# elenasolano/CS87Project-msolano2

Measured on AMD Instinct MI355X. Metric: GFLOP/s (5N·log2N/t) + % HBM roofline, fp64 complex N=2^28 @1/2/4/8 GPU, higher is better.
Workload: dtype f64; 1 GPU; config 4: one fp64 complex N=2^28 pi-FFT, P=1 workers, 1 per GPU (no data-path collective); n=268435456, workers=1, workers_per_gpu=1, batch=1, batch_per_gpu=1, local_n=268435456, passes=3, parallelism=pi-split p1 over 1 GPU(s), full=False, detail=not written: PermissionError(13, 'Permission denied')

## Files before the change

cs87project-msolano2_amd/csrc/pifft.hip:

```cpp
#ifndef _GNU_SOURCE
#define _GNU_SOURCE
#endif
#include "pifft_gather.h"
#include "pifft_kernels.h"
#include "pifft_planner.h"
#include "pifft_real.h"
#include "pifft_table.h"
#include "../../include/pifft.h"

#include <hip/hip_ext.h>
#include <hip/hip_runtime.h>

#include <math.h>
#include <stdio.h>
#include <stdlib.h>
#include <string.h>

#include <cxxabi.h>

#include <algorithm>
#include <atomic>
#include <mutex>
#include <string>
#include <vector>

using namespace pifft;

namespace {

#define HIPCHK(expr)                                                                       \
    do {                                                                                   \
        hipError_t e_ = (expr);                                                            \
        if (e_ != hipSuccess) return fail("%s failed: %s", #expr, hipGetErrorString(e_)); \
    } while (0)

bool fault_at(const char* site) {
    if (!tuning_on()) return false;
    const char* s = getenv("PIFFT_FAULT");
    const size_t n = strlen(site);
    if (!s || strncmp(s, site, n)) return false;
// ... 130 lines not shown
enum { BUF_IN = 0, BUF_OUT = 1, BUF_W = 2, BUF_TA = 3, BUF_Z = 4, NBUF = 5 };

constexpr size_t kNoTable = (size_t)-1;
struct StepTables {
    size_t r = kNoTable, lo = kNoTable, hi = kNoTable;
    size_t tree_direct = kNoTable, tree_lo = kNoTable, tree_hi = kNoTable;
};

struct Step {
    int kind = 0;
    const void* fn = nullptr;
    const PassKernel* pk = nullptr;
    dim3 grid, block;
    size_t lds = 0;
    int src = -1, dst = -2;
    uint64_t src_off = 0, dst_off = 0;
    PassArgs pa{};
    int nts = 0;
    TreeArgs ta{};
    uint64_t il_total = 0;
    uint32_t il_log_n = 0, il_log_p = 0;
    RealArgs ra{};
    StepTables tab;
    uint64_t bytes = 0;
};

}

struct pifft_plan : pifft::PlanShape {
    int device = 0, flags = 0;
    bool ilv = false;
    bool wil = false;
    bool inverse = false;
    int real = 0;
    uint64_t real_n = 0;
    size_t bytes_z = 0;
    size_t rtw_bytes = 0;
    std::vector<Step> steps;
    int tree_steps = 0, npasses = 0;
    bool fused_tree = false;
    std::vector<Step> tree_only;
    std::vector<hipEvent_t> prof_ev;
#ifdef PIFFT_WG_CLOCK
    unsigned long long* dbg_clk = nullptr;
#endif
    int prof_steps = 0, prof_used = 0, prof_mode = 0;
    int radix[8] = {0}, lines[8] = {0}, vpt[8] = {0};
    void* buf[NBUF] = {nullptr};
    size_t bytes_w = 0, bytes_ta = 0;
    void* d_tw = nullptr;
    size_t tw_bytes = 0;
    hipStream_t stream = nullptr;
    std::vector<hipEvent_t> ev;
    hipEvent_t sev[3] = {nullptr, nullptr, nullptr};
    void* d_hin = nullptr;
    void* d_hout = nullptr;
    void* d_gather = nullptr;
    std::vector<char> host_tmp;
    std::vector<int> peer_on;
    std::vector<hipStream_t> gst;
    std::vector<hipEvent_t> gdone;
    hipEvent_t gev[2] = {nullptr, nullptr};
};

namespace {

// ... 113 lines not shown
    for (auto e : p->gev)
        if (e) (void)hipEventDestroy(e);
    for (auto e : p->ev) (void)hipEventDestroy(e);
    for (auto e : p->sev)
        if (e) (void)hipEventDestroy(e);
    for (auto e : p->prof_ev) (void)hipEventDestroy(e);
    if (p->stream) (void)hipStreamDestroy(p->stream);
    delete p;
}


struct TableLayout {
    size_t tree_direct = kNoTable;
    TwoLevel tree2;
    std::vector<size_t> tw_r;
    TwoLevel pass2;
};

TableLayout layout_tables(const PlanShape& s, const PlanChoice& ch, TableBuilder& tb) {
    TableLayout tl;
    if (ch.tree_tw == TREE_TW_DIRECT || ch.tree_tw == TREE_TW_WIL_FACTORED)
        tl.tree_direct = tb.reference_omega_levels(s.n, s.lp);
    if (ch.tree_tw == TREE_TW_FACTORED || ch.tree_tw == TREE_TW_WIL_FACTORED) tl.tree2 = two_level(tb, s.n);
    tl.tw_r.resize(ch.passes.size());
    for (size_t i = 0; i < ch.passes.size(); i++) {
        size_t found = kNoTable;
        for (size_t j = 0; j < i; j++)
            if (ch.passes[j]->R == ch.passes[i]->R) found = tl.tw_r[j];
        tl.tw_r[i] = (found != kNoTable) ? found : tb.roots(ch.passes[i]->R, ch.passes[i]->R, 1);
    }
    if (ch.passes.size() > 1) tl.pass2 = two_level(tb, s.m);
    tb.align();
    return tl;
}

int assemble_steps(pifft_plan* p, const PlanChoice& ch, const TableLayout& tl) {
    const size_t esz = p->esz;
    const uint64_t ntrans = (uint64_t)p->batch * p->nq;
    const size_t npass = ch.passes.size();
    const bool need_tree = p->P > 1;
    const bool fused = ch.fused != FUSED_NONE;
    p->wil = ch.wil;
    p->ilv = ch.ilv;
    p->fused_tree = fused;
    TreeTw ttw{};
    if (need_tree) {
        ttw.h = tl.tree2.h;
        ttw.log_n = (uint32_t)p->log_n;
    }
    auto tree_tables = [&](Step& s, bool wil) {
        const bool direct = tl.tree_direct != kNoTable && !(wil && ch.tree_tw == TREE_TW_WIL_FACTORED);
        s.tab.tree_direct = direct ? tl.tree_direct : kNoTable;
        s.tab.tree_lo = direct ? kNoTable : tl.tree2.lo;
        s.tab.tree_hi = direct ? kNoTable : tl.tree2.hi;
    };

    std::vector<std::vector<Step>> chain;
    const uint64_t M = p->m;
    if (need_tree) {
        std::vector<Step> e;
        static const void* tk64[5] = {nullptr, (const void*)&k_tree<double, 1>, (const void*)&k_tree<double, 2>,
                                      (const void*)&k_tree<double, 3>, (const void*)&k_tree<double, 4>};
        static const void* tk32[5] = {nullptr, (const void*)&k_tree<float, 1>, (const void*)&k_tree<float, 2>,
                                      (const void*)&k_tree<float, 3>, (const void*)&k_tree<float, 4>};
        const int nl = (p->lp + 3) / 4;
        auto blocks_needed = [&](int t) -> uint64_t {
// ... 63 lines not shown
        const int logr = ilog2u((uint64_t)k->R);
        s.tab.r = tl.tw_r[i];
        s.tab.lo = tl.pass2.lo;
        s.tab.hi = tl.pass2.hi;
        s.pa.tw_h = tl.pass2.h;
        s.pa.in_bstride = (i == 0 && (!need_tree || fuse_here)) ? p->n : M;
        if (fuse_here) {
            s.pa.tree = ttw;
            tree_tables(s, p->wil);
            s.pa.worker = p->q0;
            s.pa.log_nq = (uint32_t)ilog2u(p->nq);
        }
        s.pa.out_bstride = M;
        s.pa.nlines = ntrans * (M >> logr);
        s.pa.log_lb = (uint32_t)(p->log_m - logr);
        s.pa.log_ns = (uint32_t)ilog2u(ns);
        s.pa.tw_shift = (uint32_t)(p->log_m - ilog2u(ns) - logr);
        s.pa.log_xg = (uint32_t)env_int((k->mode & 3) == 0 ? "PIFFT_XCD_GROUP_SINGLE" : "PIFFT_XCD_GROUP",
                                        (k->mode & 3) == 0 ? 0 : 2);
        if (last_pass) s.pa.log_xg = (uint32_t)env_int("PIFFT_LAST_XCD_GROUP", (int)s.pa.log_xg);
        if (p->wil) {
            s.pa.wil = (uint32_t)p->lp;
            s.pa.wbrev = (i + 1 == npass) ? 1u : 0u;
            s.pa.in_bstride = s.pa.out_bstride = p->n;
        }
        if (p->ilv && i + 1 == npass) {
            s.pa.ilv_log = (uint32_t)p->lp;
            s.pa.out_bstride = p->n;
            s.pa.log_xg = std::max<uint32_t>(s.pa.log_xg, (uint32_t)env_int("PIFFT_ILV_XCD_GROUP", p->lp));
        }
        s.block = dim3((unsigned)k->nt);
        s.grid = dim3((unsigned)((s.pa.nlines + (uint64_t)k->C - 1) / (uint64_t)k->C));
        s.lds = (size_t)k->lds_bytes;
        s.bytes = (!fuse_here || p->wil) ? 2 * ntrans * M * esz : (uint64_t)p->batch * p->nq * (p->n + M) * esz;
        if (i < 8) {
            p->radix[i] = k->R;
            p->lines[i] = k->C;
            p->vpt[i] = k->vpt;
        }
        ns *= (uint64_t)k->R;
        chain.push_back({s});
    }
    if (p->natural && p->P > 1 && !p->ilv && !p->wil) {
        Step s;
        s.kind = STEP_INTERLEAVE;
        s.fn = interleave_fn(p->prec, p->lp, p->n);
        s.il_total = (uint64_t)p->batch * p->n;
        s.il_log_n = (uint32_t)p->log_n;
        s.il_log_p = (uint32_t)p->lp;
        s.block = dim3(256);
        s.grid = dim3(stride_grid(interleave_threads(s.il_total, p->lp, p->prec, p->n)));
        s.bytes = 2 * s.il_total * esz;
        chain.push_back({s});
    }
    if (chain.empty()) return fail("empty plan");
    std::vector<int> dst(chain.size());
    for (size_t i = chain.size(); i-- > 0;) dst[i] = ((chain.size() - 1 - i) % 2 == 0) ? BUF_OUT : BUF_W;
    bool need_w = false;
    for (size_t i = 0; i < chain.size(); i++) {
        const int src = (i == 0) ? BUF_IN : dst[i - 1];
        if (dst[i] == BUF_W || src == BUF_W) need_w = true;
        for (auto& s : chain[i]) {
            if (s.src == -1) s.src = src;
            if (s.dst == -2) s.dst = dst[i];
            p->steps.push_back(s);
        }
// ... 465 lines not shown
            HIPCHK(hipStreamWaitEvent(d->stream, d->gdone[i], 0));
        }
        if (launch_interleave(d->d_gather, d_natural[j], N, d->P, d->batch, d->prec, d->stream)) return -1;
        HIPCHK(hipEventRecord(d->gev[1], d->stream));
        return 0;
    };
    for (int j = 0; j < np; j++) {
        if (!d_natural[j] || !enqueue(j)) continue;
        const std::string msg = g_err;
        for (int k = 0; k <= j; k++) {
            if (!d_natural[k]) continue;
            DeviceGuard g(plans[k]->device);
            for (auto st : plans[k]->gst) (void)hipStreamSynchronize(st);
            (void)hipStreamSynchronize(plans[k]->stream);
        }
        (void)hipGetLastError();
        g_err = msg;
        return -1;
    }
    double worst = 0.0;
    for (int j = 0; j < np; j++) {
        if (!d_natural[j]) continue;
        pifft_plan* d = plans[j];
        DeviceGuard g(d->device);
        HIPCHK(hipEventSynchronize(d->gev[1]));
        float t = 0.0f;
        HIPCHK(hipEventElapsedTime(&t, d->gev[0], d->gev[1]));
        worst = std::max(worst, (double)t);
    }
    if (ms) *ms = worst;
    return 0;
}

}

extern "C" {

const char* pifft_last_error(void) { return g_err.c_str(); }

int pifft_abi_version(void) { return PIFFT_ABI_VERSION; }

int pifft_gpu_count(void) {
    int n = 0;
    hipError_t e = hipGetDeviceCount(&n);
    if (e != hipSuccess) {
        fail("hipGetDeviceCount: %s", hipGetErrorString(e));
        return -1;
    }
    return n;
}

int pifft_plan_create(pifft_plan** plan, uint64_t n, uint32_t workers, uint32_t batch, int prec) {
    int dev = 0;
    if (hipGetDevice(&dev) != hipSuccess) dev = 0;
    return create(plan, n, workers, 0, workers, batch, prec, dev, PIFFT_OUT_NATURAL);
}

int pifft_plan_create_slices(pifft_plan** plan, uint64_t n, uint32_t workers, uint32_t first,
                             uint32_t count, uint32_t batch, int prec, int device, int flags) {
    return create(plan, n, workers, first, count, batch, prec, device, flags);
}

void pifft_plan_destroy(pifft_plan* plan) { release(plan); }

int pifft_plan_dry_run(uint64_t n, uint32_t workers, uint32_t first, uint32_t count, uint32_t batch, int prec,
                       int flags, pifft_plan_info* info) {
// ... 77 lines not shown
    }
    info->layout = (p->wil ? 1 : 0) | (p->ilv ? 2 : 0);
    info->num_launches = (int)p->steps.size();
    info->num_passes = p->npasses;
    info->tree_launches = p->tree_steps;
    for (int i = 0; i < 8; i++) {
        info->radix[i] = p->radix[i];
        info->lines[i] = p->lines[i];
        info->vpt[i] = p->vpt[i];
    }
    std::vector<const void*> fns;
    for (size_t i = 0; i < p->steps.size() && i < PIFFT_MAX_LAUNCH_INFO; i++) {
        info->launch_bytes[i] = p->steps[i].bytes;
        info->launch_kind[i] = p->steps[i].kind;
        size_t f = 0;
        while (f < fns.size() && fns[f] != p->steps[i].fn) f++;
        if (f == fns.size()) fns.push_back(p->steps[i].fn);
        info->launch_fn[i] = (int32_t)f;
        info->launch_mode[i] = p->steps[i].pk ? p->steps[i].pk->mode : 0;
    }
    return 0;
}

int pifft_plan_kernel_name(const pifft_plan* p, int launch, char* buf, size_t len) {
    if (!p || !buf || len == 0) return fail("NULL argument");
    if (launch < 0 || launch >= (int)p->steps.size()) return fail("launch %d out of range", launch);
    DeviceGuard g(p->device);
    const char* mangled = hipKernelNameRefByPtr(p->steps[(size_t)launch].fn, nullptr);
    if (!mangled) return fail("no kernel name for launch %d", launch);
    int st = 0;
    char* dem = abi::__cxa_demangle(mangled, nullptr, nullptr, &st);
    snprintf(buf, len, "%s", (st == 0 && dem) ? dem : mangled);
    free(dem);
    return 0;
}

int sampled_launch(int k, size_t ns) { return (k & 1) ? (int)(((size_t)k >> 1) % ns) : -1; }

int pifft_execute_device(pifft_plan* p, const void* d_in, void* d_out, void* stream) {
    if (check_buffers(p, d_in, d_out)) return -1;
    DeviceGuard g(p->device);
    hipStream_t st = (hipStream_t)stream;
    const size_t ns = p->steps.size();
    if (p->prof_used >= p->prof_steps) return launch_steps(p, d_in, d_out, st, nullptr);
    const int k = p->prof_used++;
    if (p->prof_mode == PIFFT_PROFILE_ALL) return launch_steps(p, d_in, d_out, st, &p->prof_ev[(size_t)k * 2 * ns]);
    const int li = sampled_launch(k, ns);
    for (size_t i = 0; i < ns; i++) {
        hipEvent_t* e = (int)i == li ? &p->prof_ev[(size_t)k * 2] : nullptr;
        if (launch_step(p, p->steps[i], d_in, d_out, st, e ? e[0] : nullptr, e ? e[1] : nullptr)) return -1;
    }
    return 0;
}

int pifft_launch_loop(pifft_plan* p, const int* launches, int nlaunches, int reps, const void* d_in, void* d_out,
                      void* stream, float* mean_ms) {
    if (check_buffers(p, d_in, d_out)) return -1;
    if (!launches || nlaunches < 1 || reps < 1 || !mean_ms) return fail("bad arguments");
    for (int j = 0; j < nlaunches; j++)
        if (launches[j] < 0 || (size_t)launches[j] >= p->steps.size())
            return fail("launch %d out of range (plan has %zu)", launches[j], p->steps.size());
    DeviceGuard g(p->device);
    hipStream_t st = (hipStream_t)stream;
    auto rounds = [&](int r) -> int {
        for (int k = 0; k < r; k++)
            for (int j = 0; j < nlaunches; j++)
// ... 78 lines not shown
    };
    int rc = 0;
    float best = 0.0f;
    if (timed(best)) rc = -1;
    std::vector<void*> losers;
    for (int t = 1; t < tries && rc == 0; t++) {
        void* keep = p->buf[BUF_W];
        void* fresh = nullptr;
        size_t mfree = 0, mtotal = 0;
        if (hipMemGetInfo(&mfree, &mtotal) != hipSuccess || mfree < 2 * p->bytes_w + (4ull << 30)) {
            (void)hipGetLastError();
            break;
        }
        if (hipMalloc(&fresh, p->bytes_w) != hipSuccess) {
            (void)hipGetLastError();
            break;
        }
        p->buf[BUF_W] = fresh;
        float ms = 0.0f;
        if (timed(ms)) {
            rc = -1;
            p->buf[BUF_W] = keep;
            losers.push_back(fresh);
        } else if (ms < best) {
            best = ms;
            losers.push_back(keep);
        } else {
            p->buf[BUF_W] = keep;
            losers.push_back(fresh);
        }
    }
    (void)hipStreamSynchronize(st);
    for (void* w : losers) (void)hipFree(w);
    (void)hipEventDestroy(e[0]);
    (void)hipEventDestroy(e[1]);
    if (best_ms) *best_ms = best;
    return rc;
}

int pifft_profile_start(pifft_plan* p, int steps, int mode) {
    if (!p || steps < 0) return fail("bad arguments");
    if (mode != PIFFT_PROFILE_ALL && mode != PIFFT_PROFILE_SAMPLED) return fail("unknown profile mode %d", mode);
    DeviceGuard g(p->device);
    const size_t need = (size_t)steps * 2 * (mode == PIFFT_PROFILE_ALL ? p->steps.size() : 1);
    while (p->prof_ev.size() < need) {
        hipEvent_t e;
        HIPCHK(hipEventCreateWithFlags(&e, kTimingEventFlags));
        p->prof_ev.push_back(e);
    }
    p->prof_steps = steps;
    p->prof_used = 0;
    p->prof_mode = mode;
    return 0;
}

int pifft_profile_read(pifft_plan* p, float* launch_ms_sum, int* launch_samples, int max_launches) {
    if (!p) return fail("plan is NULL");
    DeviceGuard g(p->device);
    const size_t ns = p->steps.size();
    const int used = p->prof_used;
    p->prof_steps = p->prof_used = 0;
    std::vector<float> sum(ns, 0.0f), ms;
    std::vector<int> cnt(ns, 0);
    for (int k = 0; k < used; k++) {
        if (p->prof_mode == PIFFT_PROFILE_ALL) {
            if (read_launch_ms(ns, &p->prof_ev[(size_t)k * 2 * ns], ms)) return -1;
// ... 227 lines not shown
```

cs87project-msolano2_amd/csrc/pifft_kernels.h:

```cpp
#pragma once

#include <hip/hip_runtime.h>
#include <stdint.h>

#include <type_traits>

namespace pifft {

template <typename T>
struct alignas(2 * sizeof(T)) cx {
    T re, im;
};

template <typename T>
__device__ __forceinline__ cx<T> cadd(cx<T> a, cx<T> b) {
    return {a.re + b.re, a.im + b.im};
}
template <typename T>
__device__ __forceinline__ cx<T> csub(cx<T> a, cx<T> b) {
    return {a.re - b.re, a.im - b.im};
}
template <typename T>
__device__ __forceinline__ cx<T> cmul(cx<T> a, cx<T> b) {
    return {a.re * b.re - a.im * b.im, a.re * b.im + a.im * b.re};
}
template <typename T>
__device__ __forceinline__ cx<T> mul_negi(cx<T> a) {
    return {a.im, -a.re};
}

constexpr int ilog2c(uint64_t x) { return x <= 1 ? 0 : 1 + ilog2c(x >> 1); }

template <typename T>
__device__ __forceinline__ void dft4(cx<T>& a0, cx<T>& a1, cx<T>& a2, cx<T>& a3) {
    cx<T> t0 = cadd(a0, a2), t1 = csub(a0, a2);
    cx<T> t2 = cadd(a1, a3), t3 = mul_negi(csub(a1, a3));
    a0 = cadd(t0, t2);
    a2 = csub(t0, t2);
// ... 307 lines not shown
        const int H = (1 << LP) >> (t + 1);
        if ((q >> (LP - 1 - t)) & 1) {
#pragma unroll
            for (int ml = 0; ml < H; ml++) {
                const int e = ((K + Q * ml) << t) & (NS - 1);
                const cx<T> s{(T)roots.re[e], (T)roots.im[e]};
                v[ml] = cmul(csub(v[ml], v[ml + H]), cmul(bt[t], s));
            }
        } else {
#pragma unroll
            for (int ml = 0; ml < H; ml++) v[ml] = cadd(v[ml], v[ml + H]);
        }
    }
    return v[0];
}

struct PassArgs {
    const void* in;
    void* out;
    const void* tw_r;
    const void* tw_lo;
    const void* tw_hi;
    uint64_t in_bstride;
    uint64_t out_bstride;
    uint64_t nlines;
    uint32_t log_lb;
    uint32_t log_ns;
    uint32_t tw_h;
    uint32_t tw_shift;
    TreeTw tree;
    uint32_t worker;
    uint32_t log_nq;
    uint32_t log_xg;
    uint32_t ilv_log;
    uint32_t in_pad, out_pad, out_pad_log;
    uint32_t wil, wbrev;
#ifdef PIFFT_WG_CLOCK
    unsigned long long* wg_clock;
#endif
};

#ifdef PIFFT_WG_CLOCK
#define PIFFT_WGC_WORDS 8
__device__ __forceinline__ void wgc_stamp(const PassArgs& a, int tid, int slot) {
    __builtin_amdgcn_sched_barrier(0);
    if (a.wg_clock && tid == 0) {
        __builtin_amdgcn_s_waitcnt(0);
        a.wg_clock[PIFFT_WGC_WORDS * blockIdx.x + slot] = wall_clock64();
    }
    __builtin_amdgcn_sched_barrier(0);
}
#define PIFFT_WGC(slot) wgc_stamp(a, tid, (slot))
#else
#define PIFFT_WGC(slot) ((void)0)
#endif

__device__ __forceinline__ uint64_t tile_of_block(uint32_t b, uint32_t log_xg, uint32_t nblocks) {
    if (log_xg == 0 || (nblocks & ((8u << log_xg) - 1))) return b;
    const uint32_t xcd = b & 7, slot = b >> 3, gmask = (1u << log_xg) - 1;
    return ((uint64_t)(slot >> log_xg) << (log_xg + 3)) + ((uint64_t)xcd << log_xg) + (slot & gmask);
}

template <int R, int VPT = 16>
struct PassShape {
    static constexpr int Q = R >= VPT ? VPT : (R >= 16 ? 16 : R);
    static constexpr int B = Q >= 16 ? 16 : Q;
    static constexpr int LOGB = ilog2c(B);
    static constexpr int LOGR = ilog2c(R);
    static constexpr int NSTG = LOGB ? (LOGR + LOGB - 1) / LOGB : 1;
    static constexpr int QL = 1 << (LOGR - LOGB * (NSTG - 1));
};

template <int R, int C, int VPT = 16>
struct PassCfg {
    static constexpr int NT = C * R / PassShape<R, VPT>::Q;
#ifndef PIFFT_MIN_WG_PER_CU
#define PIFFT_MIN_WG_PER_CU 2
#endif
    static constexpr int wpe = NT >= 256 ? (NT * PIFFT_MIN_WG_PER_CU) / 256 : 1;
    static constexpr int waves_per_eu = wpe > 4 ? 4 : wpe;
};

struct LdsLayout {
    int ls, xs, xm, ps, cm, cs;
};
__host__ __device__ constexpr int lds_at(LdsLayout L, int c, int r) {
    return c * L.ls + (r ^ ((r >> L.xs) & L.xm) ^ ((c & L.cm) << L.cs)) + (L.ps ? (r >> L.ps) : 0);
}
template <int R>
constexpr LdsLayout lds_default() { return LdsLayout{R + R / 16 + 1, 4, 0, 4, 0, 0}; }
template <typename T, int R, int C, int BM, int VPT>
struct LdsPick {
    static constexpr LdsLayout value = lds_default<R>();
};
// ... 730 lines not shown
    }
}

#ifndef PIFFT_PACK32
#define PIFFT_PACK32 1
#endif
template <int R, int C, int MODE, int VPT>
constexpr int first_tw_count() {
    return (MODE & 3) == 2 ? 4 * Stage<R, C, 2, 0, VPT>::U : 1;
}


#ifdef PIFFT_WG_CLOCK
#define PIFFT_WGC_ENTRY() \
    if (a.wg_clock && tid == 0) a.wg_clock[PIFFT_WGC_WORDS * blockIdx.x] = wall_clock64()
#define PIFFT_WGC_EXIT()                                                        \
    if (a.wg_clock) {                                                           \
        __builtin_amdgcn_s_waitcnt(0);       \
        __syncthreads();                                                        \
        if (tid == 0) {                                                         \
            a.wg_clock[PIFFT_WGC_WORDS * blockIdx.x + 1] = wall_clock64();      \
            a.wg_clock[PIFFT_WGC_WORDS * blockIdx.x + 2] = __smid();            \
        }                                                                       \
    }
#else
#define PIFFT_WGC_ENTRY() ((void)0)
#define PIFFT_WGC_EXIT() ((void)0)
#endif
#define PIFFT_PASS_KERNEL_BODY(SW)                                                                                   \
    extern __shared__ __attribute__((aligned(16))) unsigned char pifft_smem[];                                       \
    constexpr int Q = PassShape<R, VPT>::Q;                                                                          \
    constexpr int TWN = first_tw_count<R, C, MODE, VPT>();                                                           \
    cx<T> pre[pre_count<R, C, stage_mode(MODE), VPT>() > 0 ? pre_count<R, C, stage_mode(MODE), VPT>() : 1];          \
    uint64_t tile = tile_of_block(blockIdx.x, a.log_xg, gridDim.x);                                                  \
    T* lds = reinterpret_cast<T*>(pifft_smem);                                                                       \
    const int tid = (int)threadIdx.x;                                                                                \
    PIFFT_WGC_ENTRY();                                                                                               \
    if constexpr (VPT == 32 && std::is_same_v<T, float> && PIFFT_PACK32) {                                           \
        cx<f2> vp[PassShape<R, VPT>::Q / 2];                                                                         \
        cx<float> twp[TWN];                                                                                          \
        pass_stages_packed<R, C, MODE, NTS, 0, SW>(a, reinterpret_cast<float*>(pifft_smem), vp, tid, tile, twp);     \
        (void)pre;                                                                                                   \
        (void)lds;                                                                                                   \
    } else {                                                                                                         \
        if (a.ilv_log && a.log_lb >= (uint32_t)ilog2c(C)) {                                                          \
            const uint32_t il = a.ilv_log, ltt = a.log_lb - (uint32_t)ilog2c(C);                                     \
            const uint64_t q = tile & ((1ull << il) - 1), rest = tile >> il;                                         \
            tile = ((rest >> ltt) << (il + ltt)) + (q << ltt) + (rest & ((1ull << ltt) - 1));                        \
        }                                                                                                            \
        cx<T> v[Q];                                                                                                  \
        cx<T> twp[TWN];                                                                                              \
        pass_stages<T, R, C, MODE, NTS, LP, 0, VPT, SW>(a, lds, v, pre, tid, tile, twp);                             \
    }                                                                                                                \
    PIFFT_WGC_EXIT()

template <typename T, int R, int C, int MODE, int NTS, int LP, int VPT = 16>
__global__ __launch_bounds__((PassCfg<R, C, VPT>::NT), (pass_waves_per_eu<T, R, C, MODE, LP, VPT>()))
void k_pass(PassArgs a) {
    PIFFT_PASS_KERNEL_BODY(0);
}

template <typename T, int R, int C, int MODE, int NTS, int LP, int VPT, int SW>
__global__ __launch_bounds__((PassCfg<R, C, VPT>::NT), (pass_waves_per_eu<T, R, C, MODE, LP, VPT>()))
void k_pass_sw(PassArgs a) {
    static_assert(SW >= 1 && SW <= 3, "k_pass_sw: a swapping twin (the forward kernel is k_pass)");
    PIFFT_PASS_KERNEL_BODY(SW);
}
// ... 179 lines not shown
```

cs87project-msolano2_amd/pifft.py:

```python
from __future__ import annotations

import ctypes
import os
import subprocess

HERE = os.path.dirname(os.path.abspath(__file__))
LIB_PATH = os.environ.get("PIFFT_LIB") or os.path.join(HERE, "libpifft.so")
CLI_PATH = os.path.join(HERE, "pifft")

F32, F64 = 32, 64
OUT_NATURAL, OUT_SLICES, OUT_BITREV = 0, 1, 2
PROFILE_ALL, PROFILE_SAMPLED = 0, 1
SEPARATE_TREE = 4
INVERSE = 8
REAL_FORWARD, REAL_INVERSE = 0, 1
KIND_NAMES = {1: "tree", 2: "pass", 3: "interleave", 4: "tree+pass", 5: "r2c", 6: "c2r"}
MAX_LAUNCH_INFO = 256


class PifftError(RuntimeError):
    pass


class PlanInfo(ctypes.Structure):
# ... 33 lines not shown
    "pifft_gpu_count": (ctypes.c_int, []),
    "pifft_plan_create": (ctypes.c_int, [ctypes.POINTER(_P), ctypes.c_uint64, ctypes.c_uint32,
                                         ctypes.c_uint32, ctypes.c_int]),
    "pifft_plan_create_slices": (ctypes.c_int, [ctypes.POINTER(_P), ctypes.c_uint64, ctypes.c_uint32,
                                                ctypes.c_uint32, ctypes.c_uint32, ctypes.c_uint32,
                                                ctypes.c_int, ctypes.c_int, ctypes.c_int]),
    "pifft_plan_destroy": (None, [_P]),
    "pifft_plan_dry_run": (ctypes.c_int, [ctypes.c_uint64, ctypes.c_uint32, ctypes.c_uint32, ctypes.c_uint32,
                                          ctypes.c_uint32, ctypes.c_int, ctypes.c_int, ctypes.POINTER(PlanInfo)]),
    "pifft_plan_get_info": (ctypes.c_int, [_P, ctypes.POINTER(PlanInfo)]),
    "pifft_plan_create_real": (ctypes.c_int, [ctypes.POINTER(_P), ctypes.c_uint64, ctypes.c_uint32, ctypes.c_uint32,
                                              ctypes.c_int, ctypes.c_int, ctypes.c_int]),
    "pifft_plan_dry_run_real": (ctypes.c_int, [ctypes.c_uint64, ctypes.c_uint32, ctypes.c_uint32, ctypes.c_int,
                                               ctypes.c_int, ctypes.POINTER(PlanInfo)]),
    "pifft_plan_is_real": (ctypes.c_int, [_P]),
    "pifft_plan_kernel_name": (ctypes.c_int, [_P, ctypes.c_int, ctypes.c_char_p, ctypes.c_size_t]),
    "pifft_execute_device": (ctypes.c_int, [_P, _P, _P, _P]),
    "pifft_execute_device_timed": (ctypes.c_int, [_P, _P, _P, _P, ctypes.POINTER(ctypes.c_float),
                                                  ctypes.c_int]),
    "pifft_execute": (ctypes.c_int, [_P, _P, _P, ctypes.POINTER(ctypes.c_double),
                                     ctypes.POINTER(ctypes.c_double)]),
    "pifft_execute_group_kernel_times": (ctypes.c_int, [ctypes.POINTER(_P), ctypes.c_int,
                                                        ctypes.POINTER(ctypes.c_double),
                                                        ctypes.POINTER(ctypes.c_double)]),
    "pifft_execute_group": (ctypes.c_int, [ctypes.POINTER(_P), ctypes.c_int, _P, _P,
                                           ctypes.POINTER(ctypes.c_double), ctypes.POINTER(ctypes.c_double)]),
    "pifft_generate_device": (ctypes.c_int, [_P, ctypes.c_uint64, ctypes.c_uint64, ctypes.c_uint64,
                                             ctypes.c_uint64, ctypes.c_int, _P]),
    "pifft_interleave_device": (ctypes.c_int, [_P, _P, ctypes.c_uint64, ctypes.c_uint32, ctypes.c_uint32,
                                               ctypes.c_int, _P]),
    "pifft_tree_device": (ctypes.c_int, [_P, _P, _P, _P]),
    "pifft_profile_start": (ctypes.c_int, [_P, ctypes.c_int, ctypes.c_int]),
    "pifft_plan_tune_workspace": (ctypes.c_int, [_P, _P, _P, _P, ctypes.c_int, ctypes.POINTER(ctypes.c_float)]),
    "pifft_profile_read": (ctypes.c_int, [_P, ctypes.POINTER(ctypes.c_float), ctypes.POINTER(ctypes.c_int),
                                          ctypes.c_int]),
    "pifft_launch_loop": (ctypes.c_int, [_P, ctypes.POINTER(ctypes.c_int), ctypes.c_int, ctypes.c_int, _P, _P, _P,
                                         ctypes.POINTER(ctypes.c_float)]),
    "pifft_allgather": (ctypes.c_int, [ctypes.POINTER(_P), ctypes.c_int, ctypes.POINTER(_P), ctypes.POINTER(_P),
                                       ctypes.POINTER(ctypes.c_double)]),
    "pifft_instance_count": (ctypes.c_int, []),
    "pifft_instance_desc": (ctypes.c_int, [ctypes.c_int, ctypes.POINTER(ctypes.c_int32)]),
    "pifft_instance_found": (ctypes.c_int, [ctypes.c_int]),
    "pifft_plan_dry_run_instances": (ctypes.c_int, [ctypes.c_uint64, ctypes.c_uint32, ctypes.c_uint32,
                                                    ctypes.c_uint32, ctypes.c_uint32, ctypes.c_int, ctypes.c_int,
                                                    ctypes.POINTER(ctypes.c_int32), ctypes.c_int]),
}
SYMBOLS = tuple(_SIGS)

_lib = None


def build(quiet: bool = True) -> None:
    subprocess.run(["make", "-j16", "-C", HERE, "all"], check=True,
                   stdout=subprocess.DEVNULL if quiet else None)


def lib() -> ctypes.CDLL:
    global _lib
    if _lib is None:
        if not os.path.exists(LIB_PATH):
            raise PifftError(f"{LIB_PATH} not built (run __graft_entry__.build() or make -C {HERE})")
        try:
            import torch
        except ImportError:
            pass
        L = ctypes.CDLL(LIB_PATH)
# ... 34 lines not shown

class Plan:

    def __init__(self, n: int, workers: int = 1, batch: int = 1, prec: int = F64, *,
                 first: int = 0, count: int | None = None, device: int | None = None,
                 flags: int | None = None, inverse: bool = False):
        h = _P()
        if count is None and device is None and flags is None and first == 0 and not inverse:
            _check(lib().pifft_plan_create(ctypes.byref(h), n, workers, batch, prec), "pifft_plan_create")
        else:
            count = workers if count is None else count
            device = 0 if device is None else device
            if flags is None:
                flags = OUT_NATURAL if count == workers else OUT_SLICES
            elif flags == SEPARATE_TREE:
                flags |= OUT_NATURAL if count == workers else OUT_SLICES
            if inverse:
                flags |= INVERSE
            _check(lib().pifft_plan_create_slices(ctypes.byref(h), n, workers, first, count, batch, prec,
                                                  device, flags), "pifft_plan_create_slices")
        self._h = h
        self.info = self._info()

    def _info(self) -> PlanInfo:
        info = PlanInfo()
        _check(lib().pifft_plan_get_info(self._h, ctypes.byref(info)), "pifft_plan_get_info")
        return info

    @property
    def handle(self):
        return self._h

    def describe(self) -> dict:
        return describe_info(self.info)

    def is_real(self) -> int:
        return lib().pifft_plan_is_real(self._h)

    def kernel_name(self, launch: int) -> str:
        buf = ctypes.create_string_buffer(512)
        _check(lib().pifft_plan_kernel_name(self._h, launch, buf, len(buf)), "pifft_plan_kernel_name")
        return buf.value.decode()

    def execute_device(self, d_in: int, d_out: int, stream=None) -> None:
        _check(lib().pifft_execute_device(self._h, d_in, d_out, _stream(stream)), "pifft_execute_device")

    def execute_device_timed(self, d_in: int, d_out: int, stream=None) -> list[float]:
        n = self.info.num_launches
        buf = (ctypes.c_float * max(n, 1))()
        _check(lib().pifft_execute_device_timed(self._h, d_in, d_out, _stream(stream), buf, n),
               "pifft_execute_device_timed")
        return list(buf[:n])

    def tune_workspace(self, d_in: int, d_out: int, stream=None, tries: int = 4) -> float:
        ms = ctypes.c_float()
        _check(lib().pifft_plan_tune_workspace(self._h, d_in, d_out, _stream(stream), tries, ctypes.byref(ms)),
               "pifft_plan_tune_workspace")
        return ms.value

    def profile_start(self, steps: int, mode: int = 1) -> None:
        _check(lib().pifft_profile_start(self._h, steps, mode), "pifft_profile_start")

    def profile_read(self) -> tuple[int, list[float], list[int]]:
        n = self.info.num_launches
        buf = (ctypes.c_float * max(n, 1))()
        cnt = (ctypes.c_int * max(n, 1))()
        used = lib().pifft_profile_read(self._h, buf, cnt, n)
# ... 194 lines not shown
```

include/pifft.h:

```cpp
#ifndef PIFFT_H
#define PIFFT_H

#include <stddef.h>
#include <stdint.h>

#ifdef __cplusplus
extern "C" {
#endif

#define PIFFT_F32 32
#define PIFFT_F64 64

#define PIFFT_OUT_NATURAL 0
#define PIFFT_OUT_SLICES 1
#define PIFFT_OUT_BITREV 2

#define PIFFT_SEPARATE_TREE 4

#define PIFFT_INVERSE 8

typedef struct pifft_plan pifft_plan;

#define PIFFT_MAX_LAUNCH_INFO 256

// ... 37 lines not shown
                             uint32_t count, uint32_t batch, int prec, int device, int flags);

void pifft_plan_destroy(pifft_plan* plan);

int pifft_plan_dry_run(uint64_t n, uint32_t workers, uint32_t first, uint32_t count, uint32_t batch,
                       int prec, int flags, pifft_plan_info* info);

int pifft_plan_get_info(const pifft_plan* plan, pifft_plan_info* info);

#define PIFFT_REAL_FORWARD 0
#define PIFFT_REAL_INVERSE 1
int pifft_plan_create_real(pifft_plan** plan, uint64_t n, uint32_t workers, uint32_t batch,
                           int prec, int device, int direction);
int pifft_plan_dry_run_real(uint64_t n, uint32_t workers, uint32_t batch, int prec,
                            int direction, pifft_plan_info* info);
int pifft_plan_is_real(const pifft_plan* plan);

int pifft_instance_count(void);
int pifft_instance_desc(int i, int32_t* desc);
int pifft_instance_found(int i);
int pifft_plan_dry_run_instances(uint64_t n, uint32_t workers, uint32_t first, uint32_t count, uint32_t batch,
                                 int prec, int flags, int32_t* ids, int max_ids);

int pifft_plan_kernel_name(const pifft_plan* plan, int launch, char* buf, size_t len);

int pifft_execute_device(pifft_plan* plan, const void* d_in, void* d_out, void* stream);

int pifft_execute_device_timed(pifft_plan* plan, const void* d_in, void* d_out, void* stream,
                               float* launch_ms, int max_launches);

int pifft_plan_tune_workspace(pifft_plan* plan, const void* d_in, void* d_out, void* stream, int tries,
                              float* best_ms);

#define PIFFT_PROFILE_ALL 0
#define PIFFT_PROFILE_SAMPLED 1
int pifft_profile_start(pifft_plan* plan, int steps, int mode);
int pifft_profile_read(pifft_plan* plan, float* launch_ms_sum, int* launch_samples, int max_launches);

int pifft_launch_loop(pifft_plan* plan, const int* launches, int nlaunches, int reps, const void* d_in,
                      void* d_out, void* stream, float* mean_ms);

int pifft_execute(pifft_plan* plan, const void* host_in, void* host_out, double* ms_stage1,
                  double* ms_stage2);

int pifft_execute_group(pifft_plan** plans, int nplans, const void* host_in, void* host_out,
                        double* ms_stage1, double* ms_stage2);

int pifft_execute_group_kernel_times(pifft_plan** plans, int nplans, double* kernel_ms_stage1,
                                     double* kernel_ms_stage2);

int pifft_allgather(pifft_plan* const* plans, int nplans, const void* const* d_slices, void* const* d_natural,
                    double* ms);

int pifft_generate_device(void* d_x, uint64_t count, uint64_t n, uint64_t seed, uint64_t first,
                          int prec, void* stream);

int pifft_interleave_device(const void* d_slices, void* d_out, uint64_t n, uint32_t workers,
                            uint32_t batch, int prec, void* stream);

int pifft_tree_device(pifft_plan* plan, const void* d_in, void* d_seg, void* stream);

#ifdef __cplusplus
}
#endif

#endif
// ... 1 lines not shown
```

Baseline: 7991 GFLOP/s.

## Autotune per-pass block-to-tile order to improve memory locality

Adds a configurable permutation of block index to tile index, swapping bit fields of the group index, in the FFT pass kernels. The workspace tuner times a fixed set of candidate orders for each large pass and keeps one only if it beats the planner's default by more than the measured noise spread. The aim is to reduce HBM and cache traffic inefficiency from the order in which tiles are scheduled across XCDs. It adds a little index arithmetic per block and extra tuning time, and it only takes effect when the workspace tuner is run.

```diff
diff --git a/cs87project-msolano2_amd/csrc/pifft.hip b/cs87project-msolano2_amd/csrc/pifft.hip
--- a/cs87project-msolano2_amd/csrc/pifft.hip
+++ b/cs87project-msolano2_amd/csrc/pifft.hip
@@ -6,6 +6,7 @@
 #include "pifft_planner.h"
 #include "pifft_real.h"
 #include "pifft_table.h"
+#include "pifft_tile_candidates.h"
 #include "../../include/pifft.h"
 
 #include <hip/hip_ext.h>
@@ -202,6 +203,7 @@
     bool ilv = false;
     bool wil = false;
     bool inverse = false;
+    bool order_forced = false;
     int real = 0;
     uint64_t real_n = 0;
     size_t bytes_z = 0;
@@ -381,6 +383,33 @@
     if (ch.passes.size() > 1) tl.pass2 = two_level(tb, s.m);
     tb.align();
     return tl;
+}
+
+bool tile_order_eligible(const Step& s) {
+    return s.kind == STEP_PASS && s.pk && (s.pk->mode == 1 || s.pk->mode == 2) && !s.pa.ilv_log && !s.pa.wil;
+}
+
+bool set_tile_order(Step& s, uint32_t ts, uint32_t tw) {
+    const bool on = tile_order_eligible(s) && ts <= kTileOrderMaxS && tw <= kTileOrderMaxW &&
+                    s.pa.log_xg <= kTileOrderMaxG && tile_order_applies(s.pa.log_xg, ts, tw, s.grid.x);
+    s.pa.tile_s = on ? ts : 0;
+    s.pa.tile_w = on ? tw : 0;
+    return on;
+}
+
+int forced_tile_order(size_t pass, uint32_t& ts, uint32_t& tw) {
+    const char* c = tuning_on() ? getenv("PIFFT_TILE_ORDER") : nullptr;
+    if (!c || !*c) return 0;
+    for (size_t i = 0; i < pass; i++) {
+        const char* next = strchr(c, ',');
+        if (!next) break;
+        c = next + 1;
+    }
+    unsigned a = 0, b = 0;
+    if (sscanf(c, "%u.%u", &a, &b) != 2) return fail("PIFFT_TILE_ORDER: expected s.w[,s.w...], got '%s'", c);
+    ts = a;
+    tw = b;
+    return 1;
 }
 
 int assemble_steps(pifft_plan* p, const PlanChoice& ch, const TableLayout& tl) {
@@ -510,6 +539,15 @@
         s.block = dim3((unsigned)k->nt);
         s.grid = dim3((unsigned)((s.pa.nlines + (uint64_t)k->C - 1) / (uint64_t)k->C));
         s.lds = (size_t)k->lds_bytes;
+        {
+            uint32_t ts = 0, tw = 0;
+            const int forced = forced_tile_order(i, ts, tw);
+            if (forced < 0) return -1;
+            if (forced) {
+                p->order_forced = true;
+                set_tile_order(s, ts, tw);
+            }
+        }
         s.bytes = (!fuse_here || p->wil) ? 2 * ntrans * M * esz : (uint64_t)p->batch * p->nq * (p->n + M) * esz;
         if (i < 8) {
             p->radix[i] = k->R;
@@ -1041,6 +1079,64 @@
     return 0;
 }
 
+constexpr uint64_t kTileOrderMinBytes = 256ull << 20;
+
+int tune_tile_orders(pifft_plan* p, const void* d_in, void* d_out, hipStream_t st, hipEvent_t* e, bool* changed) {
+    auto timed = [&](const Step& s, float& ms) -> int {
+        if (launch_step(p, s, d_in, d_out, st)) return -1;
+        HIPCHK(hipEventRecord(e[0], st));
+        for (int r = 0; r < 3; r++)
+            if (launch_step(p, s, d_in, d_out, st)) return -1;
+        HIPCHK(hipEventRecord(e[1], st));
+        HIPCHK(hipEventSynchronize(e[1]));
+        HIPCHK(hipEventElapsedTime(&ms, e[0], e[1]));
+        ms /= 3.0f;
+        return 0;
+    };
+    const bool log = env_int("PIFFT_TUNE_LOG", 0) != 0;
+    for (Step& s : p->steps) {
+        if (!tile_order_eligible(s) || s.bytes < kTileOrderMinBytes) {
+            if (launch_step(p, s, d_in, d_out, st)) return -1;
+            continue;
+        }
+        set_tile_order(s, 0, 0);
+        float lo = 0.0f, hi = 0.0f;
+        for (int r = 0; r < 3; r++) {
+            float ms = 0.0f;
+            if (timed(s, ms)) return -1;
+            lo = r ? std::min(lo, ms) : ms;
+            hi = r ? std::max(hi, ms) : ms;
+        }
+        const float spread = hi - lo;
+        Step best = s;
+        float best_ms = lo - spread;
+        bool found = false;
+        for (const auto& o : kTileOrders) {
+            Step c = s;
+            float ms = 0.0f;
+            if (!set_tile_order(c, o.s, o.w)) continue;
+            if (timed(c, ms)) return -1;
+            if (ms < best_ms) best = c, best_ms = ms, found = true;
+        }
+        float again = 0.0f, base = 0.0f;
+        bool kept = false;
+        if (found) {
+            if (timed(best, again) || timed(s, base)) return -1;
+            kept = again < std::min(lo, base) - spread;
+        }
+        if (log)
+            fprintf(stderr, "pifft: tile order, launch %d: planner's %.4f-%.4f ms; best candidate (%u, %u) %.4f ms%s\n",
+                    (int)(&s - p->steps.data()), lo, hi, best.pa.tile_s, best.pa.tile_w, found ? best_ms : 0.0f,
+                    !found ? " (none beyond the spread)" : kept ? ", kept" : ", not confirmed");
+        if (kept) {
+            s = best;
+            *changed = true;
+        }
+    }
+    HIPCHK(hipStreamSynchronize(st));
+    return 0;
+}
+
 }
 
 extern "C" {
@@ -1184,6 +1280,16 @@
     char* dem = abi::__cxa_demangle(mangled, nullptr, nullptr, &st);
     snprintf(buf, len, "%s", (st == 0 && dem) ? dem : mangled);
     free(dem);
+    return 0;
+}
+
+int pifft_plan_tile_order(const pifft_plan* p, int launch, int* s, int* w) {
+    if (!p || !s || !w) return fail("NULL argument");
+    if (launch < 0 || launch >= (int)p->steps.size()) return fail("launch %d out of range", launch);
+    const Step& st = p->steps[(size_t)launch];
+    const bool pass = st.kind == STEP_PASS || st.kind == STEP_TREE_PASS;
+    *s = pass ? (int)st.pa.tile_s : 0;
+    *w = pass ? (int)st.pa.tile_w : 0;
     return 0;
 }
 
@@ -1328,6 +1434,9 @@
     }
     (void)hipStreamSynchronize(st);
     for (void* w : losers) (void)hipFree(w);
+    bool reordered = false;
+    if (rc == 0 && !p->order_forced && tune_tile_orders(p, d_in, d_out, st, e, &reordered)) rc = -1;
+    if (rc == 0 && reordered && timed(best)) rc = -1;
     (void)hipEventDestroy(e[0]);
     (void)hipEventDestroy(e[1]);
     if (best_ms) *best_ms = best;
diff --git a/cs87project-msolano2_amd/csrc/pifft_kernels.h b/cs87project-msolano2_amd/csrc/pifft_kernels.h
--- a/cs87project-msolano2_amd/csrc/pifft_kernels.h
+++ b/cs87project-msolano2_amd/csrc/pifft_kernels.h
@@ -4,6 +4,8 @@
 #include <stdint.h>
 
 #include <type_traits>
+
+#include "pifft_tile_order.h"
 
 namespace pifft {
 
@@ -377,6 +379,7 @@
     uint32_t worker;
     uint32_t log_nq;
     uint32_t log_xg;
+    uint32_t tile_s, tile_w;
     uint32_t ilv_log;
     uint32_t in_pad, out_pad, out_pad_log;
     uint32_t wil, wbrev;
@@ -400,11 +403,6 @@
 #define PIFFT_WGC(slot) ((void)0)
 #endif
 
-__device__ __forceinline__ uint64_t tile_of_block(uint32_t b, uint32_t log_xg, uint32_t nblocks) {
-    if (log_xg == 0 || (nblocks & ((8u << log_xg) - 1))) return b;
-    const uint32_t xcd = b & 7, slot = b >> 3, gmask = (1u << log_xg) - 1;
-    return ((uint64_t)(slot >> log_xg) << (log_xg + 3)) + ((uint64_t)xcd << log_xg) + (slot & gmask);
-}
 
 template <int R, int VPT = 16>
 struct PassShape {
@@ -1201,7 +1199,7 @@
     constexpr int Q = PassShape<R, VPT>::Q;                                                                          \
     constexpr int TWN = first_tw_count<R, C, MODE, VPT>();                                                           \
     cx<T> pre[pre_count<R, C, stage_mode(MODE), VPT>() > 0 ? pre_count<R, C, stage_mode(MODE), VPT>() : 1];          \
-    uint64_t tile = tile_of_block(blockIdx.x, a.log_xg, gridDim.x);                                                  \
+    uint64_t tile = tile_of_block(blockIdx.x, a.log_xg, a.tile_s, a.tile_w, gridDim.x);                              \
     T* lds = reinterpret_cast<T*>(pifft_smem);                                                                       \
     const int tid = (int)threadIdx.x;                                                                                \
     PIFFT_WGC_ENTRY();                                                                                               \
diff --git a/cs87project-msolano2_amd/csrc/pifft_tile_candidates.h b/cs87project-msolano2_amd/csrc/pifft_tile_candidates.h
--- /dev/null
+++ b/cs87project-msolano2_amd/csrc/pifft_tile_candidates.h
@@ -0,0 +1,13 @@
+#pragma once
+
+#include <stdint.h>
+
+namespace pifft {
+
+struct TileOrder {
+    uint32_t s, w;
+};
+constexpr TileOrder kTileOrders[] = {{4, 1}, {1, 7}, {2, 2}, {7, 1}, {2, 6}, {5, 7}, {6, 6}};
+static_assert(sizeof kTileOrders / sizeof kTileOrders[0] <= 7, "at most 8 orders per launch, the planner's included");
+
+}
diff --git a/cs87project-msolano2_amd/csrc/pifft_tile_order.h b/cs87project-msolano2_amd/csrc/pifft_tile_order.h
--- /dev/null
+++ b/cs87project-msolano2_amd/csrc/pifft_tile_order.h
@@ -0,0 +1,33 @@
+#pragma once
+
+#include <stdint.h>
+
+#if defined(__HIPCC__) || defined(__CUDACC__)
+#define PIFFT_HD __host__ __device__ __forceinline__
+#else
+#define PIFFT_HD inline
+#endif
+
+namespace pifft {
+
+constexpr uint32_t kTileOrderMaxS = 10, kTileOrderMaxW = 9, kTileOrderMaxG = 8;
+
+PIFFT_HD bool tile_order_applies(uint32_t g, uint32_t s, uint32_t w, uint32_t nblocks) {
+    return s != 0 && w != 0 && g + w + s < 32 && !(nblocks & ((8u << g) - 1)) &&
+           !(nblocks & ((1u << (g + w + s)) - 1));
+}
+
+PIFFT_HD uint64_t tile_of_block(uint32_t b, uint32_t log_xg, uint32_t s, uint32_t w, uint32_t nblocks) {
+    if (nblocks & ((8u << log_xg) - 1)) return b;
+    uint32_t l = b;
+    if (log_xg) {
+        const uint32_t xcd = b & 7, slot = b >> 3, gmask = (1u << log_xg) - 1;
+        l = ((slot >> log_xg) << (log_xg + 3)) + (xcd << log_xg) + (slot & gmask);
+    }
+    if (!tile_order_applies(log_xg, s, w, nblocks)) return l;
+    const uint32_t grp = l >> log_xg;
+    const uint32_t lo = grp & ((1u << w) - 1), mid = (grp >> w) & ((1u << s) - 1), hi = grp >> (w + s);
+    return (uint64_t)(l & ((1u << log_xg) - 1)) + ((uint64_t)((((hi << w) + lo) << s) + mid) << log_xg);
+}
+
+}
diff --git a/cs87project-msolano2_amd/pifft.py b/cs87project-msolano2_amd/pifft.py
--- a/cs87project-msolano2_amd/pifft.py
+++ b/cs87project-msolano2_amd/pifft.py
@@ -89,6 +89,8 @@
     "pifft_tree_device": (ctypes.c_int, [_P, _P, _P, _P]),
     "pifft_profile_start": (ctypes.c_int, [_P, ctypes.c_int, ctypes.c_int]),
     "pifft_plan_tune_workspace": (ctypes.c_int, [_P, _P, _P, _P, ctypes.c_int, ctypes.POINTER(ctypes.c_float)]),
+    "pifft_plan_tile_order": (ctypes.c_int, [_P, ctypes.c_int, ctypes.POINTER(ctypes.c_int),
+                                             ctypes.POINTER(ctypes.c_int)]),
     "pifft_profile_read": (ctypes.c_int, [_P, ctypes.POINTER(ctypes.c_float), ctypes.POINTER(ctypes.c_int),
                                           ctypes.c_int]),
     "pifft_launch_loop": (ctypes.c_int, [_P, ctypes.POINTER(ctypes.c_int), ctypes.c_int, ctypes.c_int, _P, _P, _P,
@@ -189,7 +191,15 @@
         return self._h
 
     def describe(self) -> dict:
-        return describe_info(self.info)
+        d = describe_info(self.info)
+        d["tile_order"] = [self.tile_order(i) for i in range(min(d["num_launches"], MAX_LAUNCH_INFO))]
+        return d
+
+    def tile_order(self, launch: int) -> tuple[int, int]:
+        s, w = ctypes.c_int(), ctypes.c_int()
+        _check(lib().pifft_plan_tile_order(self._h, launch, ctypes.byref(s), ctypes.byref(w)),
+               "pifft_plan_tile_order")
+        return s.value, w.value
 
     def is_real(self) -> int:
         return lib().pifft_plan_is_real(self._h)
diff --git a/include/pifft.h b/include/pifft.h
--- a/include/pifft.h
+++ b/include/pifft.h
@@ -93,6 +93,8 @@
 int pifft_plan_tune_workspace(pifft_plan* plan, const void* d_in, void* d_out, void* stream, int tries,
                               float* best_ms);
 
+int pifft_plan_tile_order(const pifft_plan* plan, int launch, int* s, int* w);
+
 #define PIFFT_PROFILE_ALL 0
 #define PIFFT_PROFILE_SAMPLED 1
 int pifft_profile_start(pifft_plan* plan, int steps, int mode);
```

New measurement: 8094 GFLOP/s, median of 5. 1.01x the previous value.
